# Tani843/Mixed_Precision_Multigrid_Solvers_for_PDEs

Measured on AMD Instinct MI355X. Metric: MDoF/s per V-cycle on 2D Poisson, higher is better.
Workload: dtype f64 (adaptive policy); 1 GPU; 2D Poisson 4097^2 adaptive fp32->fp64 (switch_threshold=1e-6), V(2,2) weighted-Jacobi omega=0.8, 11 levels, 1xMI355X; levels=11, cycle=V(2,2), smoother=jacobi, parallelism=1 GPU

## Files before the change

include/mghip.h:

```cpp
#ifndef MGHIP_H
#define MGHIP_H

#include <stdint.h>

#ifdef __cplusplus
extern "C" {
#endif

#define MG_OK 0
#define MG_ERR_INVALID_VALUE (-1)
#define MG_ERR_NO_DEVICE (-2)
#define MG_ERR_HIP (-3)
#define MG_ERR_STATE (-4)
#define MG_ERR_ALLOC (-5)

typedef enum { MG_F32 = 0, MG_F64 = 1 } mg_dtype;
typedef enum {
  MG_JACOBI = 0,
  MG_RBGS = 1,
  MG_LEXGS = 2,
  MG_ZEBRA_X = 3,
  MG_ZEBRA_Y = 4,
  MG_ZEBRA_ALT = 5
} mg_smoother_t;
// ... 19 lines not shown
  double coarse_tol;
  int32_t coarse_maxit;
  int32_t precision;
  double switch_threshold;
  double memory_threshold_gb;
  int32_t adaptive_reference_rule;
  int32_t device;
  int32_t profile;
  int32_t colour_offset;
  int32_t fused;
  int32_t tail;
  int32_t fmg_cycles;
  int32_t speculate;
  int32_t coarse_direct;
  int32_t mixed_split;
} mg_config;

typedef struct mg_stats {
  double solve_seconds;
  double h2d_seconds;
  double d2h_seconds;
  double initial_residual;
  int32_t precision_switches;
  int32_t last_coarse_sweeps;
  int32_t switch_reason;
  double fp32_floor;
} mg_stats;

typedef struct mg_handle mg_handle;

// ... 196 lines not shown
```

mixed_precision_multigrid_solvers_for_pdes_amd/_lib.py:

```python
import ctypes as C
import os

import numpy as np

from . import _build

MG_OK = 0
MG_ERR_INVALID_VALUE, MG_ERR_NO_DEVICE, MG_ERR_HIP, MG_ERR_STATE, MG_ERR_ALLOC, MG_ERR_TIMEOUT = -1, -2, -3, -4, -5, -6
MG_PLAN_PHASES = 7
PLAN_PHASE_NAMES = ("legs", "halo_copy", "halo_exchange", "coarse_allgather", "replicated_engine", "allreduce", "other")


class PlanTimeout(RuntimeError):
    """mg_plan_wait gave up (MG_ERR_TIMEOUT): the queued device work is still queued, so the process must not
    synchronise on it again -- report and leave (distributed.bench_main does, with os._exit)."""
MG_F32, MG_F64 = 0, 1
MG_JACOBI, MG_RBGS, MG_LEXGS = 0, 1, 2
MG_ZEBRA_X, MG_ZEBRA_Y, MG_ZEBRA_ALT = 3, 4, 5
MG_CYCLE_V, MG_CYCLE_W, MG_CYCLE_F = 0, 1, 2
MG_PREC_DOUBLE, MG_PREC_SINGLE, MG_PREC_MIXED_LEVELS, MG_PREC_ADAPTIVE, MG_PREC_SINGLE_MANAGED, MG_PREC_DEFECT = 0, 1, 2, 3, 4, 5

CYCLES = {"V": MG_CYCLE_V, "W": MG_CYCLE_W, "F": MG_CYCLE_F}


class MgConfig(C.Structure):
    _fields_ = [
        ("nx", C.c_int32), ("ny", C.c_int32),
        ("x0", C.c_double), ("x1", C.c_double), ("y0", C.c_double), ("y1", C.c_double),
        ("coeff", C.c_double),
        ("max_levels", C.c_int32), ("cycle", C.c_int32), ("pre", C.c_int32), ("post", C.c_int32),
        ("smoother", C.c_int32),
        ("omega", C.c_double),
        ("coarse_tol", C.c_double), ("coarse_maxit", C.c_int32),
        ("precision", C.c_int32),
        ("switch_threshold", C.c_double), ("memory_threshold_gb", C.c_double),
        ("adaptive_reference_rule", C.c_int32),
        ("device", C.c_int32), ("profile", C.c_int32), ("colour_offset", C.c_int32), ("fused", C.c_int32),
        ("tail", C.c_int32), ("fmg_cycles", C.c_int32), ("speculate", C.c_int32), ("coarse_direct", C.c_int32),
        ("mixed_split", C.c_int32),
    ]


class MgStats(C.Structure):
    _fields_ = [
        ("solve_seconds", C.c_double), ("h2d_seconds", C.c_double), ("d2h_seconds", C.c_double),
        ("initial_residual", C.c_double),
        ("precision_switches", C.c_int32), ("last_coarse_sweeps", C.c_int32),
        ("switch_reason", C.c_int32), ("fp32_floor", C.c_double),
    ]


class MgPcgStats(C.Structure):
    _fields_ = [("solve_seconds", C.c_double), ("precond_seconds", C.c_double), ("initial_residual", C.c_double),
                ("true_residual", C.c_double), ("iterations", C.c_int32), ("status", C.c_int32)]
# ... 374 lines not shown
```

mixed_precision_multigrid_solvers_for_pdes_amd/csrc/mg_engine.hip:

```cpp
#include "mg_launch.hpp"

#include <cstring>

namespace mgh {

std::string& last_error() {
  thread_local std::string msg;
  return msg;
}

static int upload(std::string* err, void* dev, int ddt, int ld, const void* host, int hdt, int nx, int ny, void* staging,
           hipStream_t st) {
  if (ddt == hdt) {
    HIPC(err, hipMemcpy2DAsync(dev, (size_t)ld * esize(ddt), host, (size_t)ny * esize(hdt), (size_t)ny * esize(hdt), nx,
                               hipMemcpyHostToDevice, st));
  } else {
    const int lds = pitch_elems(hdt, ny);
    HIPC(err, hipMemcpy2DAsync(staging, (size_t)lds * esize(hdt), host, (size_t)ny * esize(hdt), (size_t)ny * esize(hdt),
                               nx, hipMemcpyHostToDevice, st));
    d_convert(hdt, ddt, staging, dev, nx, ny, lds, ld, st);
  }
  HIPC(err, hipStreamSynchronize(st));
  return MG_OK;
}
// ... 274 lines not shown
  if ((tail2 || tail_lds) && h->cfg.tail != 0) {
    if (h->tail_direct && h->tail_minv_sigma != h->sigma) { const int rc = build_coarse_inverse(h); if (rc != MG_OK) return rc; }
    if (tail2) return tail2_launch(h, zero_u);
    launch_tail(h, zero_u);
    return MG_OK;
  }
  if (l == L - 1) {
    coarse_solve(h, l, zero_u);
    return MG_OK;
  }
  Level& c = h->lv[l + 1];
  const int dc = h->level_dtype(l + 1);
  const bool fine = (l == 0);
  const int sm = h->cfg.smoother;
  LegGeom g = leg_geom(h, l, dt, dc);
  if (part != kPartBack) {
    StageTimer tm(h, &f, 0);
    if (h->cfg.pre > 2 && zero_u) { (void)hipMemsetAsync(f.u[dt], 0, bytes, h->stream); zero_u = false; }
    extra_sweeps(h, f, dt, g, h->cfg.pre - 2);
    g.nsweep = std::min(2, h->cfg.pre);
    d_down(sm, dt, dc, f.u[dt], f.rhs[dt], f.t[dt], c.rhs[dc], g, zero_u, h->stream);
    std::swap(f.u[dt], f.t[dt]);
  }
  for (int k = 0, n = h->visits(l); k < n && part != kPartBack; ++k) {
    const int rc = cycle_fused(h, l + 1, k == 0);
    if (rc != MG_OK) return rc;
  }
  if (part != kPartFront) {
    StageTimer tm(h, &f, 2);
    const bool want_norm = fine && h->cfg.post <= 2 && h->cfg.precision != MG_PREC_DEFECT;
    g.nsweep = std::min(2, h->cfg.post);
    const int n = d_up(sm, dt, dc, h->grid_dtype, f.u[dt], f.rhs[dt], f.t[dt], c.u[dc], h->partials, g, want_norm, h->stream);
    if (n < 0) return MG_ERR_INVALID_VALUE;
    std::swap(f.u[dt], f.t[dt]);
    if (fine) h->norm_partials = want_norm ? n : 0;
    extra_sweeps(h, f, dt, g, h->cfg.post - 2);
  }
// ... 244 lines not shown
int mg_create(const mg_config* cfg, mg_handle** out) {
  if (!cfg || !out) return fail(nullptr, MG_ERR_INVALID_VALUE, "mg_create: NULL argument");
  *out = nullptr;
  if (cfg->nx < 3 || cfg->ny < 3)
    return fail(nullptr, MG_ERR_INVALID_VALUE, "Grid must have at least 3 points in each direction");
  if (cfg->cycle < MG_CYCLE_V || cfg->cycle > MG_CYCLE_F) return fail(nullptr, MG_ERR_INVALID_VALUE, "unknown cycle type");
  if (cfg->smoother < MG_JACOBI || cfg->smoother > MG_ZEBRA_ALT) return fail(nullptr, MG_ERR_INVALID_VALUE, "unknown smoother");
  if (is_zebra(cfg->smoother) && cfg->colour_offset != 0)
    return fail(nullptr, MG_ERR_INVALID_VALUE, "line smoothers serve a single domain: colour_offset must be 0");
  if (is_zebra(cfg->smoother) && !line_shape_ok(cfg->smoother == MG_ZEBRA_Y ? 3 : cfg->nx, cfg->smoother == MG_ZEBRA_X ? 3 : cfg->ny))
    return fail(nullptr, MG_ERR_INVALID_VALUE, "line smoothers: lines of more than 16384 cells do not fit a workgroup's LDS");
  if (cfg->precision < MG_PREC_DOUBLE || cfg->precision > MG_PREC_DEFECT) return fail(nullptr, MG_ERR_INVALID_VALUE, "unknown precision policy");
  if (cfg->pre < 0 || cfg->post < 0 || cfg->max_levels < 1 || cfg->coarse_maxit < 1)
    return fail(nullptr, MG_ERR_INVALID_VALUE, "negative sweep count / max_levels < 1 / coarse_maxit < 1");
  if (!(cfg->x1 > cfg->x0) || !(cfg->y1 > cfg->y0)) return fail(nullptr, MG_ERR_INVALID_VALUE, "empty domain");

  int ndev = 0;
  int rc = mg_device_count(&ndev);
  if (rc != MG_OK) return rc;
  if (ndev <= 0 || cfg->device < 0 || cfg->device >= ndev) return fail(nullptr, MG_ERR_NO_DEVICE, "no such HIP device");
  HIPC(nullptr, hipSetDevice(cfg->device));

  mg_handle* h = new mg_handle();
  h->cfg = *cfg;
  h->grid_dtype = (cfg->precision == MG_PREC_SINGLE) ? MG_F32 : MG_F64;
  h->phase = MG_F64;
  int nx = cfg->nx, ny = cfg->ny;
  for (int level = 0; level < cfg->max_levels; ++level) {
    if (level > 0) {
      if ((nx - 1) % 2 != 0 || (ny - 1) % 2 != 0) break;
// ... 345 lines not shown
```

mixed_precision_multigrid_solvers_for_pdes_amd/csrc/mg_launch.hip:

```cpp
#include "mg_launch.hpp"
#include "mg_rb_kernels.hpp"

#include <cstring>

namespace mgh {

int pitch_elems(int dt, int ny) {
  const size_t bytes = ((size_t)ny * esize(dt) + 511) / 512 * 512;
  return (int)(bytes / esize(dt));
}

template <typename T>
mg::TileGeom make_geom(int nx, int ny, int ld, bool interior_only) {
  using S = mg::TileShape<T>;
  mg::TileGeom g;
  g.nx = nx; g.ny = ny; g.ld = ld;
  g.nyv = std::min(ld, (ny + S::N - 1) / S::N * S::N);
  g.i_org = interior_only ? 1 : 0;
  const int rows = interior_only ? nx - 2 : nx;
  const int cols = interior_only ? ny - 1 : ny;
  const int tiles_i = (rows + mg::kTI - 1) / mg::kTI;
  g.tiles_j = (cols + S::TJ - 1) / S::TJ;
  g.ntiles = tiles_i * g.tiles_j;
  return g;
}

size_t max_partials(int nx, int ny) {
  const long long tj = (ny + 63) / 64 + 1;
  const int ti_min = std::min(mg::kTI, std::min(mg::kFusedTI, std::min(mg::kFusedTISmall, mg::kFusedTITiny)));
  const long long ti = (nx + ti_min - 1) / ti_min + 1;
  return (size_t)std::max<long long>(2048, ti * tj);
}

static int grid_for(long long work_items) {
  long long b = (work_items + mg::kBlock - 1) / mg::kBlock;
  return (int)std::max<long long>(1, std::min<long long>(b, 256 * 16));
}
bool use_rb(const LegGeom& g) { return g.rb == 2 || (g.rb == 1 && (long long)g.nx * g.ny > 1100LL * 1100LL); }

static bool rb_stream(const LegGeom& g, size_t esz) {
  static const int force = exp_env("MG_RB_NT", -1);
  if (force >= 0) return force != 0;
  return (size_t)g.nx * g.ld * esz > (size_t)100 << 20;
}

static bool jacobi_rb(int dt, const void* u, const void* rhs, void* out, int nx, int ny, int ld, double hx, double hy, double omega,
               hipStream_t st, double sigma) {
  static const int on = exp_env("MG_JACOBI_RB", 1);
  LegGeom g;
  g.nx = nx; g.ny = ny; g.ld = ld; g.hx = hx; g.hy = hy; g.omega = omega; g.nsweep = 1; g.fine = true;
  g.sigma = sigma; g.rb = 1;
  if (!on || !use_rb(g) || !rb_stream(g, esize(dt))) return false;
  d_sweeps(MG_JACOBI, dt, u, rhs, out, g, st);
// ... 204 lines not shown
  mg::FusedArgs a = fused_args<T, HALO, mg::kFusedTI>(g, use_div);
  const int tiles_i = (g.nx - 2 + S::TI - 1) / S::TI;
  a.tiles_j = (g.ny - 1 + S::TJ - 1) / S::TJ;
  a.ntiles = tiles_i * a.tiles_j;
  return a;
}
#if !defined(MG_EXPERIMENTS) && (defined(MG_EXP_VAR_W) || defined(MG_EXP_RB_W))
#error "MG_EXP_* switches need -DMG_EXPERIMENTS (a measurement build, never the shipped library)"
#endif
#ifndef MG_EXP_VAR_W
#define MG_EXP_VAR_W 8
#endif
#ifndef MG_EXP_RB_W
#define MG_EXP_RB_W ((SM == mg::kSmRbgs && sizeof(T) == 8) ? 8 : 4)
#endif

enum LegKind { kLegDown, kLegUpNorm, kLegUp, kLegSweeps };
enum LegFamily { kLdsTiled, kRegBlocked };

template <int LEG, int FAM, typename T, typename TX, typename TC, int SM, int TI, int W = 0, int RPT = 0, bool VAR = false>
int launch_leg(const void* u, const void* rhs, void* out, const void* coarse, double* partials, const LegGeom& g, bool zero_init,
               hipStream_t st) {
  constexpr bool PROLONG = LEG == kLegUpNorm || LEG == kLegUp;
  constexpr int POST = LEG == kLegDown ? mg::kPostRestrict : LEG == kLegUpNorm ? mg::kPostNorm : mg::kPostNone;
  constexpr int HALO = 2 * mg::sweep_halo(SM) + (LEG == kLegDown ? 2 : LEG == kLegUpNorm ? 1 : 0);
  const Coef c = coefs(g.hx, g.hy, g.sigma);
  mg::FusedArgs a;
  const double coeff = LEG == kLegSweeps ? 0.0 : g.coeff;
  if constexpr (FAM == kRegBlocked) {
    a = rb_args<T, HALO, W, RPT>(g, !c.pow2);
    if (pow2_stencil(c, sizeof(T) == 8, g.acoef, g.sigma, coeff)) { a.pow2 = 1; a.neg_coeff_a = -(coeff * c.ihx2); }
  } else a = fused_args<T, HALO, TI>(g, !c.pow2);
  const bool nt = FAM == kRegBlocked && rb_stream(g, sizeof(T));
  auto pick = [&](auto zero) {
    constexpr bool Z = decltype(zero)::value;
    if constexpr (FAM == kRegBlocked) {
      return nt ? mg::rb_leg_kernel<T, HALO, PROLONG, POST, Z, TX, TC, 2, SM, W, RPT, VAR>
                : mg::rb_leg_kernel<T, HALO, PROLONG, POST, Z, TX, TC, 1, SM, W, RPT, VAR>;
    } else {
      return g.acoef ? mg::fused_jacobi_kernel<T, HALO, PROLONG, POST, Z, TX, TC, 0, SM, TI, true>
           : g.fine ? mg::fused_jacobi_kernel<T, HALO, PROLONG, POST, Z, TX, TC, 1, SM, TI>
                    : mg::fused_jacobi_kernel<T, HALO, PROLONG, POST, Z, TX, TC, 0, SM, TI>;
    }
  };
  auto k = pick(std::false_type());
  if constexpr (LEG == kLegDown) if (zero_init) k = pick(std::true_type());
  hipLaunchKernelGGL(k, dim3(a.ntiles), dim3(FAM == kRegBlocked ? W * 64 : mg::kFusedBlock), 0, st, (const T*)u, (const T*)rhs,
                     (T*)out, PROLONG ? (const TX*)coarse : nullptr, POST == mg::kPostRestrict ? (TX*)coarse : nullptr,
                     POST == mg::kPostNorm ? partials : nullptr, a, (T)c.ihx2, (T)c.ihy2, (T)c.invD, (T)c.diag, (T)g.omega,
                     (T)(1.0 - g.omega), (T)coeff, (const T*)g.acoef, (T)g.sigma, (const T*)g.rdiag);
  return POST == mg::kPostNorm ? a.ntiles : 0;
}
template <int LEG, typename T, typename TX, typename TC, int SM>
int launch_leg_sized(const void* u, const void* rhs, void* out, const void* coarse, double* partials, const LegGeom& g,
                     bool zero_init, hipStream_t st) {
  if (use_rb(g))
    return g.acoef ? launch_leg<LEG, kRegBlocked, T, TX, TC, SM, 0, MG_EXP_VAR_W, 4, true>(u, rhs, out, coarse, partials, g, zero_init, st)
                   : launch_leg<LEG, kRegBlocked, T, TX, TC, SM, 0, MG_EXP_RB_W, 8, false>(u, rhs, out, coarse, partials, g, zero_init, st);
  if (tiny_tiles(g)) return launch_leg<LEG, kLdsTiled, T, TX, TC, SM, mg::kFusedTITiny>(u, rhs, out, coarse, partials, g, zero_init, st);
  if (small_tiles(g, SM)) return launch_leg<LEG, kLdsTiled, T, TX, TC, SM, mg::kFusedTISmall>(u, rhs, out, coarse, partials, g, zero_init, st);
  return launch_leg<LEG, kLdsTiled, T, TX, TC, SM, mg::kFusedTI>(u, rhs, out, coarse, partials, g, zero_init, st);
}

template <typename T, typename TX, typename TC, int SM>
int launch_span_rb(const void* u, const void* rhs, void* out_mid, void* out_next, const void* e_c, void* rhs_c, double* partials,
                   const LegGeom& g, int nsweep_pre, hipStream_t st) {
  constexpr int W = 8, RPT = 8;
  constexpr int HALO = 4 * mg::sweep_halo(SM) + 2;
  const Coef c = coefs(g.hx, g.hy, g.sigma);
  mg::FusedArgs a = rb_args<T, HALO, W, RPT>(g, !c.pow2);
// ... 191 lines not shown
```

mixed_precision_multigrid_solvers_for_pdes_amd/csrc/mg_launch.hpp:

```cpp
#pragma once

#include "mg_host.hpp"

namespace mgh {

int pitch_elems(int dt, int ny);
size_t max_partials(int nx, int ny);

void d_jacobi(int dt, const void* u, const void* rhs, void* out, int nx, int ny, int ld, double hx, double hy,
              double omega, hipStream_t st, bool fine = false, double sigma = 0.0);
void d_rbgs_colour(int dt, void* u, const void* rhs, int nx, int ny, int ld, double hx, double hy, double omega,
                   int colour, int poff, hipStream_t st, bool fine = false, double sigma = 0.0);
void d_residual(int dt, const void* u, const void* f, void* r, int nx, int ny, int ld, double hx, double hy,
                double coeff, hipStream_t st, bool fine = false, double sigma = 0.0);
int d_residual_norm(int dt, const void* u, const void* f, double* partials, int nx, int ny, int ld, double hx,
                    double hy, double coeff, hipStream_t st, bool fine = false, double sigma = 0.0);
int d_sumsq(int dt, const void* x, double* partials, int ld, int i_lo, int i_hi, int j_lo, int j_hi, hipStream_t st);
void launch_reduce(const double* partials, int n, double* out, hipStream_t st, mg::HostMailbox* mailbox = nullptr,
                   unsigned long long seq = 0);
void d_restrict_sub(int di, int dout, const void* fine, void* coarse, int ldf, int nxc, int nyc, int ldc, int sides,
                    hipStream_t st);
void d_restrict(int di, int dout, const void* fine, void* coarse, int nxf, int nyf, int ldf, int ldc, hipStream_t st);
int d_prolong_sub(bool add, int dc, int df, int dcomp, const void* e, void* u, int nxf, int nyf, int ldf, int nxc, int nyc,
                  int ldc, int sides, hipStream_t st);
// ... 13 lines not shown
void d_inject_ring(int di, int dout, const void* fine, void* coarse, int nxf, int nyf, int ldf, int nxc, int nyc, int ldc,
                   hipStream_t st, int sides = mg::kAllSides, int ci_off = 0, int cj_off = 0);

struct LegGeom {
  int nx = 0, ny = 0, ld = 0, nxc = 0, nyc = 0, ldc = 0;
  double hx = 0, hy = 0, omega = 0, coeff = 0;
  int nsweep = 0, poff = 0;
  bool fine = false;
  int ci_off = 0, cj_off = 0, sides = mg::kAllSides;
  int ni_lo = -1, ni_hi = -1, nj_lo = -1, nj_hi = -1;
  int select = 0, in_i_lo = 0, in_i_hi = 0, in_j_lo = 0, in_j_hi = 0;
  double sigma = 0.0;
  const void* acoef = nullptr;
  const void* rdiag = nullptr;
  int rb = 0;
};
bool use_rb(const LegGeom& g);

int d_span(int dt, int dcomp, const void* u, const void* rhs, void* out_mid, void* out_next, const void* e_c, void* rhs_c,
           double* partials, const LegGeom& g, int nsweep_pre, hipStream_t st, int sm = MG_JACOBI);
void d_down(int sm, int dt, int dx, const void* u, const void* rhs, void* out, void* rhs_c, const LegGeom& g, bool zero_init,
            hipStream_t st);
int d_up(int sm, int dt, int dx, int dcomp, const void* u, const void* rhs, void* out, const void* e_c, double* partials,
         const LegGeom& g, bool norm, hipStream_t st);
void d_sweeps(int sm, int dt, const void* u, const void* rhs, void* out, const LegGeom& g, hipStream_t st);

constexpr size_t kTailPoolLimit = 150 * 1024;
size_t tail_pool_bytes(const mg_handle* h, int k, size_t esz, size_t esz_last);
int tail_set_attrs(size_t bytes);
void launch_tail(mg_handle* h, bool zero_top);

// ... 7 lines not shown
```

mixed_precision_multigrid_solvers_for_pdes_amd/csrc/mg_rb_kernels.hpp:

```cpp
#pragma once

#include "mg_kernels.hpp"

namespace mg {

#ifndef MG_RB_HL_MIN
#define MG_RB_HL_MIN 4
#endif
template <typename T, int HALO, int W, int RPT> struct RbShape {
  static constexpr int N = VecW<T>::N;
  static constexpr int HL = (MG_RB_HL_MIN <= 2 && 2 * N >= HALO) ? 2 : ((HALO + N - 1) / N > 4 ? (HALO + N - 1) / N : 4);
  static constexpr int RI = W * RPT;
  static constexpr int RJ = 64 * N;
  static constexpr int TI = RI - 2 * HALO;
  static constexpr int TJ = (64 - 2 * HL) * N;
  static_assert(TI > 0 && TI % 2 == 0, "tile height must be even (coarse rows sit on every other tile row)");
  static_assert(RPT % 2 == 0, "rows per wave must be even (row parities are compile-time constants per strip row)");
  static_assert(HL * N >= HALO, "lateral halo too narrow");
};

#ifndef MG_RB_NT_MODE
#define MG_RB_NT_MODE 3
#endif
template <typename T> __device__ __forceinline__ T dpp_from_lower_lane(T x);
// ... 78 lines not shown
  }
  static __device__ __forceinline__ Pack<float> resid(const Pack<float>& mid, const Pack<float>& dn, const Pack<float>& up, float left,
                                                      float right, const Pack<float>& f, float ihx2, float ihy2, float D, float coeff,
                                                      bool , float) {
    const f2 m0 = {mid.v[0], mid.v[1]}, m1 = {mid.v[2], mid.v[3]};
    const f2 sx0 = f2{dn.v[0], dn.v[1]} + f2{up.v[0], up.v[1]}, sx1 = f2{dn.v[2], dn.v[3]} + f2{up.v[2], up.v[3]};
    const f2 sy0 = f2{mid.v[1], mid.v[2]} + f2{left, mid.v[0]}, sy1 = f2{mid.v[3], right} + f2{mid.v[1], mid.v[2]};
    const f2 au0 = coeff * ((sx0 * ihx2 + sy0 * ihy2) - m0 * D), au1 = coeff * ((sx1 * ihx2 + sy1 * ihy2) - m1 * D);
    const f2 r0 = f2{f.v[0], f.v[1]} - au0, r1 = f2{f.v[2], f.v[3]} - au1;
    Pack<float> r;
    r.v[0] = r0.x; r.v[1] = r0.y; r.v[2] = r1.x; r.v[3] = r1.y;
    return r;
  }
};

template <typename T, int W>
__device__ __forceinline__ void rb_exchange(Pack<T>* __restrict__ xb, int w, int lane, const Pack<T>& top, const Pack<T>& bottom,
                                            Pack<T>& above, Pack<T>& below) {
  xb[(w * 2 + 0) * 64 + lane] = top;
  xb[(w * 2 + 1) * 64 + lane] = bottom;
  __syncthreads();
  above = (w > 0) ? xb[((w - 1) * 2 + 1) * 64 + lane] : zero_pack<T>();
  below = (w < W - 1) ? xb[((w + 1) * 2 + 0) * 64 + lane] : zero_pack<T>();
}

template <typename T, bool NONTEMPORAL> __device__ __forceinline__ Pack<T> ldg_global(const T* p) {
  typedef int v4i __attribute__((ext_vector_type(4)));
  const __attribute__((address_space(1))) v4i* g = (const __attribute__((address_space(1))) v4i*)p;
  const v4i v = NONTEMPORAL ? __builtin_nontemporal_load(g) : *g;
  return *reinterpret_cast<const Pack<T>*>(&v);
// ... 37 lines not shown
        pr += DR; pc += DC;
        if (pc >= PW) { pc -= PW; pr += 1; }
      }
    }
    __builtin_amdgcn_sched_barrier(0);
  }
  __device__ __forceinline__ void store(TX* __restrict__ patch) const {
    asm volatile("" ::: "memory");
    __builtin_amdgcn_sched_barrier(0);
#pragma unroll
    for (int t = 0; t < TRIPS; ++t) patch[(int)threadIdx.x + (valid(t) ? t : t - 1) * NTHR] = v[t];
    __builtin_amdgcn_sched_barrier(0);
  }
};

template <typename T, int HALO, bool PROLONG, int POST, bool ZERO_INIT, typename TX, typename TC, int SM, int W, int RPT, bool INT, int NT,
          bool VAR, int SPAN = 0>
__device__ __forceinline__ void rb_leg_body(const T* __restrict__ u, const T* __restrict__ rhs, T* __restrict__ out,
                                            const TX* __restrict__ e_coarse, TX* __restrict__ rhs_coarse,
                                            double* __restrict__ partials, const FusedArgs& a, T ihx2, T ihy2, T invD, T D, T omega,
                                            T one_m_omega, T coeff, Pack<T>* __restrict__ xbuf, TX* __restrict__ patch,
                                            double* __restrict__ red, int i0, int j0, const T* __restrict__ acoef, T sigma,
                                            const T* __restrict__ rdiag, T* __restrict__ out2 = nullptr) {
  static_assert(SPAN == 0 || (PROLONG && POST == kPostRestrict && !ZERO_INIT), "a spanning leg is an up leg followed by a down leg");
  using S = RbShape<T, HALO, W, RPT>;
  constexpr int N = S::N;
  constexpr int PH = S::RI / 2 + 2, PW = S::RJ / 2 + 2;
  constexpr int kRowPar = (1 - HALO) & 1;
  const int ri0 = i0 - HALO, rj0 = j0 - S::HL * N;
  const int lane = threadIdx.x & 63, w = __builtin_amdgcn_readfirstlane(threadIdx.x >> 6);
  const int gj0 = rj0 + lane * N;
  const int r_base = w * RPT;
  const bool col_in = INT || (gj0 >= 0 && gj0 < a.nyv);
  const bool pow2 = INT && !VAR && a.pow2 != 0;
  const T neg_coeff_a = (T)a.neg_coeff_a;

  const int pic0 = (ri0 >> 1) + a.ci_off, pjc0 = (rj0 >> 1) + a.cj_off;
  auto staging_loop = [&]() {
    for (int idx = threadIdx.x; idx < PH * PW; idx += W * 64) {
// ... 50 lines not shown
#pragma unroll
    for (int k = 0; k < RPT; ++k) {
      const Pack<T> up = (k > 0) ? A[k > 0 ? k - 1 : 0] : a_above;
      const Pack<T> dn = (k < RPT - 1) ? A[k < RPT - 1 ? k + 1 : 0] : a_below;
      const T left = dpp_from_lower_lane<T>(A[k].v[N - 1]);
      const T right = dpp_from_upper_lane<T>(A[k].v[0]);
#pragma unroll
      for (int e = 0; e < N; ++e) {
        av[VAR ? k : 0].v[e] = T(0.5) * (A[k].v[e] + up.v[e]);
        if (k == RPT - 1) av[VAR ? RPT : 0].v[e] = T(0.5) * (A[k].v[e] + dn.v[e]);
        ah[VAR ? k : 0][VAR ? e : 0] = T(0.5) * (A[k].v[e] + ((e == 0) ? left : A[k].v[e > 0 ? e - 1 : 0]));
      }
      ah[VAR ? k : 0][VAR ? N : 0] = T(0.5) * (A[k].v[N - 1] + right);
    }
  }
  if (PROLONG) {
    __syncthreads();
    using TS = typename std::conditional<(sizeof(TC) > sizeof(T)), TC, T>::type;
    if (INT) {
      constexpr int M = N / 2 + 1;
      const TX* pl = patch + (r_base / 2) * PW + lane * (N / 2);
#pragma unroll
      for (int k = 0; k < RPT; ++k) {
        const bool iodd = ((kRowPar + k) & 1) != 0;
        const int pr = (k + kRowPar) >> 1;
        TC av[M], bv[M];
#pragma unroll
        for (int m = 0; m < M; ++m) {
          av[m] = (TC)pl[pr * PW + m];
          bv[m] = iodd ? (TC)pl[(pr + 1) * PW + m] : TC(0);
        }
#pragma unroll
        for (int e = 0; e < N; ++e) {
          const int m = e >> 1;
          TC val;
          if ((e & 1) == 0) val = iodd ? TC(0.5) * (av[m] + bv[m]) : av[m];
          else val = iodd ? TC(0.25) * (((av[m] + av[m + 1]) + bv[m]) + bv[m + 1]) : TC(0.5) * (av[m] + av[m + 1]);
          U[k].v[e] = (T)((TS)U[k].v[e] + (TS)val);
        }
      }
    } else {
      const TX* pe = patch - ((ptrdiff_t)pic0 * PW + pjc0);
#pragma unroll
      for (int k = 0; k < RPT; ++k) {
        const int gi = ri0 + r_base + k;
        if (gi >= 0 && gi < a.nx && col_in) {
          TC val[N];
          bool ok[N];
          prolong_vec<TX, TC, N>(pe, PW, a.nxc, a.nyc, gi, gj0, a.nx, a.ny, a.sides, val, ok, a.ci_off, a.cj_off);
#pragma unroll
          for (int e = 0; e < N; ++e)
            if (ok[e]) U[k].v[e] = (T)((TS)U[k].v[e] + (TS)val[e]);
        } else {
          F[k] = zero_pack<T>();
          U[k] = zero_pack<T>();
        }
      }
    }
  }

  int stage = 0;
  auto run_sweeps = [&](int nsw) {
  const int npass = (SM == kSmRbgs) ? 2 * nsw : nsw;
  for (int s = 0; s < npass; ++s, ++stage) {
    Pack<T> above, below;
    rb_exchange<T, W>(xbuf + (size_t)(stage & 1) * W * 2 * 64, w, lane, U[0], U[RPT - 1], above, below);
    const int colour = s & 1;
    static_assert(N % 2 == 0 && RPT % 2 == 0, "strip rows / lane cells must be even for a workgroup-uniform colour parity");
    const int par0 = (ri0 + rj0 + a.colour_offset) & 1;
    auto pass = [&](auto qp) {
      constexpr int QP = decltype(qp)::value;
      Pack<T> prev = above;
#pragma unroll
      for (int k = 0; k < RPT; ++k) {
        const int r = r_base + k, gi = ri0 + r;
// ... 24 lines not shown
            const T sx = aip * dn.v[e] + aim * prev.v[e], sy = ajp * ea + ajm * wv;
            const T un = (F[k].v[e] + (ihx2 * sx + ihy2 * sy)) * RD[VAR ? k : 0].v[e];
            const T res = one_m_omega * mid.v[e] + omega * un;
            const int gj = gj0 + e;
            if (INT || (gj >= 1 && gj < a.ny - 1)) o.v[e] = res;
          }
        }
        U[k] = o;
        prev = (SM == kSmRbgs) ? o : mid;
      }
    };
    if (SM == kSmRbgs && ((par0 + colour) & 1) != 0) pass(std::integral_constant<int, 1>{});
    else pass(std::integral_constant<int, 0>{});
  }
  };
  run_sweeps(a.nsweep);

  const bool lane_in_tile = lane >= S::HL && lane < 64 - S::HL;
  auto store_tile = [&](T* __restrict__ dst) {
#pragma unroll
    for (int k = 0; k < RPT; ++k) {
      const int r = r_base + k, gi = ri0 + r;
      if (r >= HALO && r < HALO + S::TI && lane_in_tile && (INT || (gi < a.nx && gj0 < a.nyv))) {
        if (NT & 1) stg_nt(dst + (size_t)gi * a.ld + gj0, U[k]); else stg(dst + (size_t)gi * a.ld + gj0, U[k]);
      }
    }
  };
  if (SPAN != 2) store_tile(out);
  if (POST == kPostNone) return;

  Pack<T> R[RPT];
  double acc = 0.0;
  auto residual = [&](auto norm_stage) {
    constexpr bool NORM = decltype(norm_stage)::value;
    Pack<T> above, below;
    rb_exchange<T, W>(xbuf + (size_t)(stage & 1) * W * 2 * 64, w, lane, U[0], U[RPT - 1], above, below);
    ++stage;
#pragma unroll
    for (int k = 0; k < RPT; ++k) {
      const int r = r_base + k, gi = ri0 + r;
      const Pack<T> up = (k > 0) ? U[k - 1] : above;
      const Pack<T> mid = U[k];
      const Pack<T> dn = (k < RPT - 1) ? U[k + 1] : below;
// ... 70 lines not shown
      if (!INT && (ic < 1 || ic > a.nxc - 2 || fi < 1 || fi > a.nx - 2)) continue;
#pragma unroll
      for (int e = 0; e < N; e += 2) {
        const int fj = gj0 + e, jc = (fj >> 1) + a.cj_off;
        if (!INT && (jc < 1 || jc > a.nyc - 2 || fj < 1 || fj > a.ny - 2)) continue;
        const T NWv = (e == 0) ? nw0 : up.v[e > 0 ? e - 1 : 0], Wv = (e == 0) ? w0 : mid.v[e > 0 ? e - 1 : 0],
                SWv = (e == 0) ? sw0 : dn.v[e > 0 ? e - 1 : 0];
        const T corners = ((NWv + up.v[e + 1]) + SWv) + dn.v[e + 1];
        const T edges = ((up.v[e] + dn.v[e]) + Wv) + mid.v[e + 1];
        rhs_coarse[(size_t)ic * a.ldc + jc] = (TX)((T(1.0 / 16.0) * corners + T(1.0 / 8.0) * edges) + T(1.0 / 4.0) * mid.v[e]);
      }
    }
  }
}

template <typename T, int HALO, bool PROLONG, int POST, bool ZERO_INIT, typename TX, typename TC, int TAG, int SM, int W, int RPT,
          bool VAR = false>
__global__ __launch_bounds__(W * 64, (VAR && sizeof(T) == 8) ? 4 : 1) void rb_leg_kernel(
    const T* __restrict__ u, const T* __restrict__ rhs, T* __restrict__ out,
    const TX* __restrict__ e_coarse,
    TX* __restrict__ rhs_coarse,
    double* __restrict__ partials,
    FusedArgs a, T ihx2, T ihy2, T invD, T D, T omega, T one_m_omega, T coeff,
    const T* __restrict__ acoef,
    T sigma,
    const T* __restrict__ rdiag) {
  using S = RbShape<T, HALO, W, RPT>;
  constexpr int N = S::N;
  constexpr int kNT = (TAG == 2) ? MG_RB_NT_MODE : 0;
  constexpr int PH = S::RI / 2 + 2, PW = S::RJ / 2 + 2;
  constexpr size_t kXBytes = (size_t)2 * W * 2 * 64 * sizeof(Pack<T>);
// ... 55 lines not shown
  const int per_band = a.band * a.tiles_j;
  const int b = L / per_band, within = L - b * per_band;
  const int rows = min(a.band, tiles_i - b * a.band);
  const int tj = within / rows, ti = b * a.band + (within - tj * rows);
  const int i0 = 1 + ti * S::TI, j0 = tj * S::TJ;
  const int ri0 = i0 - HALO, rj0 = j0 - S::HL * N;
  bool interior = ri0 >= 1 && ri0 + S::RI <= a.nx - 1 && rj0 >= 1 && rj0 + S::RJ <= a.ny - 1;
  {
    const int pic0 = (ri0 >> 1) + a.ci_off, pjc0 = (rj0 >> 1) + a.cj_off;
    interior = interior && pic0 >= 0 && pic0 + PH <= a.nxc && pjc0 >= 0 && pjc0 + PW <= a.nyc;
  }
  interior = interior && i0 >= a.ni_lo && i0 + S::TI <= a.ni_hi && j0 >= a.nj_lo && j0 + S::TJ <= a.nj_hi;
  interior = interior && ((i0 + 1) >> 1) + a.ci_off >= 1 && ((i0 + S::TI - 1) >> 1) + a.ci_off <= a.nxc - 2 &&
             (j0 >> 1) + a.cj_off >= 1 && ((j0 + S::TJ - 2) >> 1) + a.cj_off <= a.nyc - 2;
  if (interior)
    rb_leg_body<T, HALO, true, kPostRestrict, false, TX, TC, SM, W, RPT, true, kNT, false, SPAN>(
        u, rhs, out_mid, e_coarse, rhs_coarse, partials, a, ihx2, ihy2, invD, D, omega, one_m_omega, coeff, xbuf, patch, red, i0, j0,
        nullptr, T(0), nullptr, out_next);
  else
    rb_leg_body<T, HALO, true, kPostRestrict, false, TX, TC, SM, W, RPT, false, kNT, false, SPAN>(
        u, rhs, out_mid, e_coarse, rhs_coarse, partials, a, ihx2, ihy2, invD, D, omega, one_m_omega, coeff, xbuf, patch, red, i0, j0,
        nullptr, T(0), nullptr, out_next);
}

}
```

mixed_precision_multigrid_solvers_for_pdes_amd/engine.py:

```python
import ctypes as C

import numpy as np

from . import _lib


def _direct_code(coarse_direct):
    import os
    if coarse_direct is None:
        coarse_direct = {"0": False, "1": True}.get(os.environ.get("MG_COARSE_DIRECT", "auto"), "auto")
    if isinstance(coarse_direct, str):
        if coarse_direct != "auto":
            raise ValueError(f"coarse_direct: True, False, 'auto' or None, not {coarse_direct!r}")
        return -1
    return int(bool(coarse_direct))


class MultigridEngine:

    def __init__(self, nx, ny, domain=(0.0, 1.0, 0.0, 1.0), coeff=-1.0, max_levels=4, cycle="V", pre=2, post=2,
                 smoother=_lib.MG_JACOBI, omega=0.8, coarse_tol=1e-12, coarse_maxit=1000,
                 precision=_lib.MG_PREC_DOUBLE, switch_threshold=1e-6, memory_threshold_gb=4.0,
                 adaptive_reference_rule=False, device=0, profile=False, colour_offset=0, fused=2, tail=True, speculate=True, fmg_cycles=0,
                 mixed_split=0, coarse_direct=None):
        lib = _lib.load()
        if isinstance(cycle, str):
            if cycle not in _lib.CYCLES:
                raise ValueError(f"unknown cycle type {cycle!r}")
            cycle = _lib.CYCLES[cycle]
        cfg = _lib.MgConfig(int(nx), int(ny), float(domain[0]), float(domain[1]), float(domain[2]), float(domain[3]),
                            float(coeff), int(max_levels), int(cycle), int(pre), int(post), int(smoother),
                            float(omega), float(coarse_tol), int(coarse_maxit), int(precision),
                            float(switch_threshold), float(memory_threshold_gb), int(bool(adaptive_reference_rule)),
                            int(device), int(bool(profile)), int(colour_offset), int(fused), int(tail), int(fmg_cycles), (2 if speculate is True else int(speculate)),
                            _direct_code(coarse_direct), int(mixed_split))
        self.cfg = cfg
        self._h = C.c_void_p(None)
        _lib.check(lib.mg_create(C.byref(cfg), C.byref(self._h)))
        self._lib = lib
        n = C.c_int(0)
        self._check(lib.mg_num_levels(self._h, C.byref(n)))
        self.num_levels = n.value
        self.shapes = []
        for l in range(self.num_levels):
            a, b = C.c_int(0), C.c_int(0)
            self._check(lib.mg_level_shape(self._h, l, C.byref(a), C.byref(b)))
            self.shapes.append((a.value, b.value))
        self.nx, self.ny = int(nx), int(ny)

    def _check(self, rc):
# ... 151 lines not shown
```

Before: 83770 MDoF/s.

## Recompute zero-start pre-smoothing in up leg instead of storing it

```diff
diff --git a/include/mghip.h b/include/mghip.h
--- a/include/mghip.h
+++ b/include/mghip.h
@@ -57,6 +57,7 @@
   int32_t speculate;
   int32_t coarse_direct;
   int32_t mixed_split;
+  int32_t zero_start_legs;
 } mg_config;
 
 typedef struct mg_stats {
diff --git a/mixed_precision_multigrid_solvers_for_pdes_amd/_lib.py b/mixed_precision_multigrid_solvers_for_pdes_amd/_lib.py
--- a/mixed_precision_multigrid_solvers_for_pdes_amd/_lib.py
+++ b/mixed_precision_multigrid_solvers_for_pdes_amd/_lib.py
@@ -37,7 +37,7 @@
         ("adaptive_reference_rule", C.c_int32),
         ("device", C.c_int32), ("profile", C.c_int32), ("colour_offset", C.c_int32), ("fused", C.c_int32),
         ("tail", C.c_int32), ("fmg_cycles", C.c_int32), ("speculate", C.c_int32), ("coarse_direct", C.c_int32),
-        ("mixed_split", C.c_int32),
+        ("mixed_split", C.c_int32), ("zero_start_legs", C.c_int32),
     ]
 
 
diff --git a/mixed_precision_multigrid_solvers_for_pdes_amd/csrc/mg_engine.hip b/mixed_precision_multigrid_solvers_for_pdes_amd/csrc/mg_engine.hip
--- a/mixed_precision_multigrid_solvers_for_pdes_amd/csrc/mg_engine.hip
+++ b/mixed_precision_multigrid_solvers_for_pdes_amd/csrc/mg_engine.hip
@@ -312,13 +312,16 @@
   const bool fine = (l == 0);
   const int sm = h->cfg.smoother;
   LegGeom g = leg_geom(h, l, dt, dc);
+  const bool recompute = l >= 1 && zero_u && part == kPartFull && h->cfg.pre >= 1 && h->cfg.pre <= 2 && recompute_ok(sm, g) &&
+                         h->cfg.zero_start_legs == 0;
+  if (recompute) g.recompute_pre = h->cfg.pre;
   if (part != kPartBack) {
     StageTimer tm(h, &f, 0);
     if (h->cfg.pre > 2 && zero_u) { (void)hipMemsetAsync(f.u[dt], 0, bytes, h->stream); zero_u = false; }
     extra_sweeps(h, f, dt, g, h->cfg.pre - 2);
     g.nsweep = std::min(2, h->cfg.pre);
     d_down(sm, dt, dc, f.u[dt], f.rhs[dt], f.t[dt], c.rhs[dc], g, zero_u, h->stream);
-    std::swap(f.u[dt], f.t[dt]);
+    if (!recompute) std::swap(f.u[dt], f.t[dt]);
   }
   for (int k = 0, n = h->visits(l); k < n && part != kPartBack; ++k) {
     const int rc = cycle_fused(h, l + 1, k == 0);
@@ -593,6 +596,7 @@
   if (cfg->pre < 0 || cfg->post < 0 || cfg->max_levels < 1 || cfg->coarse_maxit < 1)
     return fail(nullptr, MG_ERR_INVALID_VALUE, "negative sweep count / max_levels < 1 / coarse_maxit < 1");
   if (!(cfg->x1 > cfg->x0) || !(cfg->y1 > cfg->y0)) return fail(nullptr, MG_ERR_INVALID_VALUE, "empty domain");
+  if (cfg->zero_start_legs < 0 || cfg->zero_start_legs > 1) return fail(nullptr, MG_ERR_INVALID_VALUE, "zero_start_legs: 0 or 1");
 
   int ndev = 0;
   int rc = mg_device_count(&ndev);
diff --git a/mixed_precision_multigrid_solvers_for_pdes_amd/csrc/mg_launch.hip b/mixed_precision_multigrid_solvers_for_pdes_amd/csrc/mg_launch.hip
--- a/mixed_precision_multigrid_solvers_for_pdes_amd/csrc/mg_launch.hip
+++ b/mixed_precision_multigrid_solvers_for_pdes_amd/csrc/mg_launch.hip
@@ -37,6 +37,7 @@
   return (int)std::max<long long>(1, std::min<long long>(b, 256 * 16));
 }
 bool use_rb(const LegGeom& g) { return g.rb == 2 || (g.rb == 1 && (long long)g.nx * g.ny > 1100LL * 1100LL); }
+bool recompute_ok(int sm, const LegGeom& g) { return sm == MG_JACOBI && use_rb(g) && !g.acoef; }
 
 static bool rb_stream(const LegGeom& g, size_t esz) {
   static const int force = exp_env("MG_RB_NT", -1);
@@ -271,37 +272,47 @@
 #ifndef MG_EXP_RB_W
 #define MG_EXP_RB_W ((SM == mg::kSmRbgs && sizeof(T) == 8) ? 8 : 4)
 #endif
+#if !defined(MG_EXPERIMENTS) && defined(MG_EXP_RB_PAIR_W)
+#error "MG_EXP_* switches need -DMG_EXPERIMENTS (a measurement build, never the shipped library)"
+#endif
+#ifndef MG_EXP_RB_PAIR_W
+#define MG_EXP_RB_PAIR_W MG_EXP_RB_W
+#endif
 
 enum LegKind { kLegDown, kLegUpNorm, kLegUp, kLegSweeps };
 enum LegFamily { kLdsTiled, kRegBlocked };
 
-template <int LEG, int FAM, typename T, typename TX, typename TC, int SM, int TI, int W = 0, int RPT = 0, bool VAR = false>
+template <int LEG, int FAM, typename T, typename TX, typename TC, int SM, int TI, int W = 0, int RPT = 0, bool VAR = false,
+          bool RECOMP = false>
 int launch_leg(const void* u, const void* rhs, void* out, const void* coarse, double* partials, const LegGeom& g, bool zero_init,
                hipStream_t st) {
+  static_assert(!RECOMP || (FAM == kRegBlocked && !VAR && (LEG == kLegDown || LEG == kLegUp)), "the recomputing pair: constant coefficients");
   constexpr bool PROLONG = LEG == kLegUpNorm || LEG == kLegUp;
   constexpr int POST = LEG == kLegDown ? mg::kPostRestrict : LEG == kLegUpNorm ? mg::kPostNorm : mg::kPostNone;
-  constexpr int HALO = 2 * mg::sweep_halo(SM) + (LEG == kLegDown ? 2 : LEG == kLegUpNorm ? 1 : 0);
+  constexpr int HALO = 2 * mg::sweep_halo(SM) + (LEG == kLegDown ? 2 : LEG == kLegUpNorm ? 1 : 0) +
+                       (RECOMP && PROLONG ? 2 * mg::sweep_halo(SM) : 0) - (RECOMP ? mg::sweep_halo(SM) : 0);
   const Coef c = coefs(g.hx, g.hy, g.sigma);
   mg::FusedArgs a;
   const double coeff = LEG == kLegSweeps ? 0.0 : g.coeff;
   if constexpr (FAM == kRegBlocked) {
     a = rb_args<T, HALO, W, RPT>(g, !c.pow2);
     if (pow2_stencil(c, sizeof(T) == 8, g.acoef, g.sigma, coeff)) { a.pow2 = 1; a.neg_coeff_a = -(coeff * c.ihx2); }
+    if (RECOMP && PROLONG) a.nsweep2 = std::min(2, g.recompute_pre);
   } else a = fused_args<T, HALO, TI>(g, !c.pow2);
   const bool nt = FAM == kRegBlocked && rb_stream(g, sizeof(T));
   auto pick = [&](auto zero) {
-    constexpr bool Z = decltype(zero)::value;
+    constexpr int Z = decltype(zero)::value;
     if constexpr (FAM == kRegBlocked) {
       return nt ? mg::rb_leg_kernel<T, HALO, PROLONG, POST, Z, TX, TC, 2, SM, W, RPT, VAR>
                 : mg::rb_leg_kernel<T, HALO, PROLONG, POST, Z, TX, TC, 1, SM, W, RPT, VAR>;
     } else {
-      return g.acoef ? mg::fused_jacobi_kernel<T, HALO, PROLONG, POST, Z, TX, TC, 0, SM, TI, true>
-           : g.fine ? mg::fused_jacobi_kernel<T, HALO, PROLONG, POST, Z, TX, TC, 1, SM, TI>
-                    : mg::fused_jacobi_kernel<T, HALO, PROLONG, POST, Z, TX, TC, 0, SM, TI>;
+      return g.acoef ? mg::fused_jacobi_kernel<T, HALO, PROLONG, POST, Z != 0, TX, TC, 0, SM, TI, true>
+           : g.fine ? mg::fused_jacobi_kernel<T, HALO, PROLONG, POST, Z != 0, TX, TC, 1, SM, TI>
+                    : mg::fused_jacobi_kernel<T, HALO, PROLONG, POST, Z != 0, TX, TC, 0, SM, TI>;
     }
   };
-  auto k = pick(std::false_type());
-  if constexpr (LEG == kLegDown) if (zero_init) k = pick(std::true_type());
+  auto k = pick(std::integral_constant<int, RECOMP ? 2 : 0>());
+  if constexpr (LEG == kLegDown && !RECOMP) if (zero_init) k = pick(std::integral_constant<int, 1>());
   hipLaunchKernelGGL(k, dim3(a.ntiles), dim3(FAM == kRegBlocked ? W * 64 : mg::kFusedBlock), 0, st, (const T*)u, (const T*)rhs,
                      (T*)out, PROLONG ? (const TX*)coarse : nullptr, POST == mg::kPostRestrict ? (TX*)coarse : nullptr,
                      POST == mg::kPostNorm ? partials : nullptr, a, (T)c.ihx2, (T)c.ihy2, (T)c.invD, (T)c.diag, (T)g.omega,
@@ -311,6 +322,9 @@
 template <int LEG, typename T, typename TX, typename TC, int SM>
 int launch_leg_sized(const void* u, const void* rhs, void* out, const void* coarse, double* partials, const LegGeom& g,
                      bool zero_init, hipStream_t st) {
+  if constexpr (SM == mg::kSmJacobi && (LEG == kLegDown || LEG == kLegUp))
+    if (g.recompute_pre > 0 && recompute_ok(MG_JACOBI, g) && (LEG == kLegUp || zero_init))
+      return launch_leg<LEG, kRegBlocked, T, TX, TC, SM, 0, MG_EXP_RB_PAIR_W, 8, false, true>(u, rhs, out, coarse, partials, g, zero_init, st);
   if (use_rb(g))
     return g.acoef ? launch_leg<LEG, kRegBlocked, T, TX, TC, SM, 0, MG_EXP_VAR_W, 4, true>(u, rhs, out, coarse, partials, g, zero_init, st)
                    : launch_leg<LEG, kRegBlocked, T, TX, TC, SM, 0, MG_EXP_RB_W, 8, false>(u, rhs, out, coarse, partials, g, zero_init, st);
diff --git a/mixed_precision_multigrid_solvers_for_pdes_amd/csrc/mg_launch.hpp b/mixed_precision_multigrid_solvers_for_pdes_amd/csrc/mg_launch.hpp
--- a/mixed_precision_multigrid_solvers_for_pdes_amd/csrc/mg_launch.hpp
+++ b/mixed_precision_multigrid_solvers_for_pdes_amd/csrc/mg_launch.hpp
@@ -51,7 +51,9 @@
   const void* acoef = nullptr;
   const void* rdiag = nullptr;
   int rb = 0;
+  int recompute_pre = 0;
 };
+bool recompute_ok(int sm, const LegGeom& g);
 bool use_rb(const LegGeom& g);
 
 int d_span(int dt, int dcomp, const void* u, const void* rhs, void* out_mid, void* out_next, const void* e_c, void* rhs_c,
diff --git a/mixed_precision_multigrid_solvers_for_pdes_amd/csrc/mg_rb_kernels.hpp b/mixed_precision_multigrid_solvers_for_pdes_amd/csrc/mg_rb_kernels.hpp
--- a/mixed_precision_multigrid_solvers_for_pdes_amd/csrc/mg_rb_kernels.hpp
+++ b/mixed_precision_multigrid_solvers_for_pdes_amd/csrc/mg_rb_kernels.hpp
@@ -116,6 +116,18 @@
   }
 };
 
+template <typename T, int N>
+__device__ __forceinline__ Pack<T> relax_from_zero(const Pack<T>& f, T invD, T D, T omega, T z, bool use_div) {
+  Pack<T> res;
+#pragma unroll
+  for (int e = 0; e < N; ++e) {
+    const T t = f.v[e] + T(0);
+    const T un = use_div ? t / D : t * invD;
+    res.v[e] = z + omega * un;
+  }
+  return res;
+}
+
 template <typename T, int W>
 __device__ __forceinline__ void rb_exchange(Pack<T>* __restrict__ xb, int w, int lane, const Pack<T>& top, const Pack<T>& bottom,
                                             Pack<T>& above, Pack<T>& below) {
@@ -183,7 +195,7 @@
   }
 };
 
-template <typename T, int HALO, bool PROLONG, int POST, bool ZERO_INIT, typename TX, typename TC, int SM, int W, int RPT, bool INT, int NT,
+template <typename T, int HALO, bool PROLONG, int POST, int ZERO_INIT, typename TX, typename TC, int SM, int W, int RPT, bool INT, int NT,
           bool VAR, int SPAN = 0>
 __device__ __forceinline__ void rb_leg_body(const T* __restrict__ u, const T* __restrict__ rhs, T* __restrict__ out,
                                             const TX* __restrict__ e_coarse, TX* __restrict__ rhs_coarse,
@@ -192,6 +204,8 @@
                                             double* __restrict__ red, int i0, int j0, const T* __restrict__ acoef, T sigma,
                                             const T* __restrict__ rdiag, T* __restrict__ out2 = nullptr) {
   static_assert(SPAN == 0 || (PROLONG && POST == kPostRestrict && !ZERO_INIT), "a spanning leg is an up leg followed by a down leg");
+  static_assert(ZERO_INIT >= 0 && ZERO_INIT <= 2 && (ZERO_INIT != 2 || (!VAR && SM == kSmJacobi)), "ZERO_INIT 2: weighted Jacobi, constant coefficients");
+  constexpr bool kRecompute = PROLONG && ZERO_INIT == 2, kNoStore = !PROLONG && ZERO_INIT == 2;
   using S = RbShape<T, HALO, W, RPT>;
   constexpr int N = S::N;
   constexpr int PH = S::RI / 2 + 2, PW = S::RJ / 2 + 2;
@@ -272,51 +286,6 @@
       ah[VAR ? k : 0][VAR ? N : 0] = T(0.5) * (A[k].v[N - 1] + right);
     }
   }
-  if (PROLONG) {
-    __syncthreads();
-    using TS = typename std::conditional<(sizeof(TC) > sizeof(T)), TC, T>::type;
-    if (INT) {
-      constexpr int M = N / 2 + 1;
-      const TX* pl = patch + (r_base / 2) * PW + lane * (N / 2);
-#pragma unroll
-      for (int k = 0; k < RPT; ++k) {
-        const bool iodd = ((kRowPar + k) & 1) != 0;
-        const int pr = (k + kRowPar) >> 1;
-        TC av[M], bv[M];
-#pragma unroll
-        for (int m = 0; m < M; ++m) {
-          av[m] = (TC)pl[pr * PW + m];
-          bv[m] = iodd ? (TC)pl[(pr + 1) * PW + m] : TC(0);
-        }
-#pragma unroll
-        for (int e = 0; e < N; ++e) {
-          const int m = e >> 1;
-          TC val;
-          if ((e & 1) == 0) val = iodd ? TC(0.5) * (av[m] + bv[m]) : av[m];
-          else val = iodd ? TC(0.25) * (((av[m] + av[m + 1]) + bv[m]) + bv[m + 1]) : TC(0.5) * (av[m] + av[m + 1]);
-          U[k].v[e] = (T)((TS)U[k].v[e] + (TS)val);
-        }
-      }
-    } else {
-      const TX* pe = patch - ((ptrdiff_t)pic0 * PW + pjc0);
-#pragma unroll
-      for (int k = 0; k < RPT; ++k) {
-        const int gi = ri0 + r_base + k;
-        if (gi >= 0 && gi < a.nx && col_in) {
-          TC val[N];
-          bool ok[N];
-          prolong_vec<TX, TC, N>(pe, PW, a.nxc, a.nyc, gi, gj0, a.nx, a.ny, a.sides, val, ok, a.ci_off, a.cj_off);
-#pragma unroll
-          for (int e = 0; e < N; ++e)
-            if (ok[e]) U[k].v[e] = (T)((TS)U[k].v[e] + (TS)val[e]);
-        } else {
-          F[k] = zero_pack<T>();
-          U[k] = zero_pack<T>();
-        }
-      }
-    }
-  }
-
   int stage = 0;
   auto run_sweeps = [&](int nsw) {
   const int npass = (SM == kSmRbgs) ? 2 * nsw : nsw;
@@ -371,7 +340,72 @@
     else pass(std::integral_constant<int, 0>{});
   }
   };
-  run_sweeps(a.nsweep);
+  auto sweeps_from_zero = [&](int nsw) {
+    if (nsw < 1) return;
+    const T z = one_m_omega * T(0);
+#pragma unroll
+    for (int k = 0; k < RPT; ++k) {
+      const int gi = ri0 + r_base + k;
+      const Pack<T> res = relax_from_zero<T, N>(F[k], invD, D, omega, z, a.use_div != 0);
+      if (INT || (gi >= 1 && gi < a.nx - 1)) {
+#pragma unroll
+        for (int e = 0; e < N; ++e) {
+          const int gj = gj0 + e;
+          if (INT || (gj >= 1 && gj < a.ny - 1)) U[k].v[e] = res.v[e];
+        }
+      }
+    }
+    run_sweeps(nsw - 1);
+  };
+  if constexpr (kRecompute) sweeps_from_zero(a.nsweep2);
+
+  if (PROLONG) {
+    __syncthreads();
+    using TS = typename std::conditional<(sizeof(TC) > sizeof(T)), TC, T>::type;
+    if (INT) {
+      constexpr int M = N / 2 + 1;
+      const TX* pl = patch + (r_base / 2) * PW + lane * (N / 2);
+#pragma unroll
+      for (int k = 0; k < RPT; ++k) {
+        const bool iodd = ((kRowPar + k) & 1) != 0;
+        const int pr = (k + kRowPar) >> 1;
+        TC av[M], bv[M];
+#pragma unroll
+        for (int m = 0; m < M; ++m) {
+          av[m] = (TC)pl[pr * PW + m];
+          bv[m] = iodd ? (TC)pl[(pr + 1) * PW + m] : TC(0);
+        }
+#pragma unroll
+        for (int e = 0; e < N; ++e) {
+          const int m = e >> 1;
+          TC val;
+          if ((e & 1) == 0) val = iodd ? TC(0.5) * (av[m] + bv[m]) : av[m];
+          else val = iodd ? TC(0.25) * (((av[m] + av[m + 1]) + bv[m]) + bv[m + 1]) : TC(0.5) * (av[m] + av[m + 1]);
+          U[k].v[e] = (T)((TS)U[k].v[e] + (TS)val);
+        }
+      }
+    } else {
+      const TX* pe = patch - ((ptrdiff_t)pic0 * PW + pjc0);
+#pragma unroll
+      for (int k = 0; k < RPT; ++k) {
+        const int gi = ri0 + r_base + k;
+        if (gi >= 0 && gi < a.nx && col_in) {
+          TC val[N];
+          bool ok[N];
+          prolong_vec<TX, TC, N>(pe, PW, a.nxc, a.nyc, gi, gj0, a.nx, a.ny, a.sides, val, ok, a.ci_off, a.cj_off);
+#pragma unroll
+          for (int e = 0; e < N; ++e)
+            if (ok[e]) U[k].v[e] = (T)((TS)U[k].v[e] + (TS)val[e]);
+        } else {
+          F[k] = zero_pack<T>();
+          U[k] = zero_pack<T>();
+        }
+      }
+    }
+  }
+
+  if constexpr (kNoStore) sweeps_from_zero(a.nsweep);
+  else run_sweeps(a.nsweep);
 
   const bool lane_in_tile = lane >= S::HL && lane < 64 - S::HL;
   auto store_tile = [&](T* __restrict__ dst) {
@@ -383,7 +417,7 @@
       }
     }
   };
-  if (SPAN != 2) store_tile(out);
+  if (SPAN != 2 && !kNoStore) store_tile(out);
   if (POST == kPostNone) return;
 
   Pack<T> R[RPT];
@@ -484,7 +518,7 @@
   }
 }
 
-template <typename T, int HALO, bool PROLONG, int POST, bool ZERO_INIT, typename TX, typename TC, int TAG, int SM, int W, int RPT,
+template <typename T, int HALO, bool PROLONG, int POST, int ZERO_INIT, typename TX, typename TC, int TAG, int SM, int W, int RPT,
           bool VAR = false>
 __global__ __launch_bounds__(W * 64, (VAR && sizeof(T) == 8) ? 4 : 1) void rb_leg_kernel(
     const T* __restrict__ u, const T* __restrict__ rhs, T* __restrict__ out,
@@ -570,11 +604,11 @@
   interior = interior && ((i0 + 1) >> 1) + a.ci_off >= 1 && ((i0 + S::TI - 1) >> 1) + a.ci_off <= a.nxc - 2 &&
              (j0 >> 1) + a.cj_off >= 1 && ((j0 + S::TJ - 2) >> 1) + a.cj_off <= a.nyc - 2;
   if (interior)
-    rb_leg_body<T, HALO, true, kPostRestrict, false, TX, TC, SM, W, RPT, true, kNT, false, SPAN>(
+    rb_leg_body<T, HALO, true, kPostRestrict, 0, TX, TC, SM, W, RPT, true, kNT, false, SPAN>(
         u, rhs, out_mid, e_coarse, rhs_coarse, partials, a, ihx2, ihy2, invD, D, omega, one_m_omega, coeff, xbuf, patch, red, i0, j0,
         nullptr, T(0), nullptr, out_next);
   else
-    rb_leg_body<T, HALO, true, kPostRestrict, false, TX, TC, SM, W, RPT, false, kNT, false, SPAN>(
+    rb_leg_body<T, HALO, true, kPostRestrict, 0, TX, TC, SM, W, RPT, false, kNT, false, SPAN>(
         u, rhs, out_mid, e_coarse, rhs_coarse, partials, a, ihx2, ihy2, invD, D, omega, one_m_omega, coeff, xbuf, patch, red, i0, j0,
         nullptr, T(0), nullptr, out_next);
 }
diff --git a/mixed_precision_multigrid_solvers_for_pdes_amd/engine.py b/mixed_precision_multigrid_solvers_for_pdes_amd/engine.py
--- a/mixed_precision_multigrid_solvers_for_pdes_amd/engine.py
+++ b/mixed_precision_multigrid_solvers_for_pdes_amd/engine.py
@@ -22,7 +22,7 @@
                  smoother=_lib.MG_JACOBI, omega=0.8, coarse_tol=1e-12, coarse_maxit=1000,
                  precision=_lib.MG_PREC_DOUBLE, switch_threshold=1e-6, memory_threshold_gb=4.0,
                  adaptive_reference_rule=False, device=0, profile=False, colour_offset=0, fused=2, tail=True, speculate=True, fmg_cycles=0,
-                 mixed_split=0, coarse_direct=None):
+                 mixed_split=0, coarse_direct=None, zero_start_legs=0):
         lib = _lib.load()
         if isinstance(cycle, str):
             if cycle not in _lib.CYCLES:
@@ -33,7 +33,7 @@
                             float(omega), float(coarse_tol), int(coarse_maxit), int(precision),
                             float(switch_threshold), float(memory_threshold_gb), int(bool(adaptive_reference_rule)),
                             int(device), int(bool(profile)), int(colour_offset), int(fused), int(tail), int(fmg_cycles), (2 if speculate is True else int(speculate)),
-                            _direct_code(coarse_direct), int(mixed_split))
+                            _direct_code(coarse_direct), int(mixed_split), int(zero_start_legs))
         self.cfg = cfg
         self._h = C.c_void_p(None)
         _lib.check(lib.mg_create(C.byref(cfg), C.byref(self._h)))
```

Result: no change. 85180 MDoF/s, median of 4 (+1.7%).
